# TritonDataCenter/manatee

Hardware: NVIDIA H100
Metric: snapshot_stream_gibs (higher is better)
Workload: dtype u8 / u32->u64 (mod 2^64)

## Files before the change

manatee_b200/csrc/kernels_lz4.cuh:

```cuda
#pragma once
#include <stdint.h>
#include <cuda_runtime.h>
#ifdef LZ4_PROF
#include <cstdio>
#endif
#include "../../include/manatee_gpu.h"

namespace mtz {

#define LZ4_MINMATCH     4
#define LZ4_LASTLITERALS 5
#define LZ4_MFLIMIT      12
#define LZ4_MINLENGTH    13
#define LZ4_MAXDIST      65535
#define LZ4_64KLIMIT     ((1 << 16) + (LZ4_MFLIMIT - 1))
#define LZ4_SKIPSTRENGTH 6

__device__ __forceinline__ uint32_t ld_u8(const uint8_t *p) { return *p; }

#define LZ4_SEQ_NONE 0xffffffffu
__device__ __forceinline__ uint64_t lz4_seq_pack(uint32_t m, uint32_t off, uint32_t ml)
{
	return (uint64_t)m | ((uint64_t)off << 24) | ((uint64_t)ml << 40);
}

__device__ __forceinline__ int32_t warp_lz4_decode(const uint8_t *__restrict__ src,
    uint32_t psize, uint8_t *__restrict__ dst, uint32_t lsize, int lane,
    uint64_t *__restrict__ seq = nullptr, uint32_t seq_cap = 0, uint32_t *seq_n = nullptr)
{
	uint32_t ns = 0;
	if (seq_n != nullptr && lane == 0) *seq_n = LZ4_SEQ_NONE;
	if (psize < 4u) return MTZ_ECODEC;
	const uint32_t clen = (ld_u8(src) << 24) | (ld_u8(src + 1) << 16) | (ld_u8(src + 2) << 8) | ld_u8(src + 3);
	if ((uint64_t)clen + 4u > psize || clen == 0u) return MTZ_ECODEC;
	const uint8_t *in = src + 4;
	uint32_t ip = 0, op = 0;
	const uint32_t iend = clen;

	for (;;) {
		if (ip >= iend) return MTZ_ECODEC;
		const uint32_t tok = ld_u8(in + ip++);
		uint32_t len = tok >> 4;
		if (len == 15u) {
			uint32_t s;
			do {
				if (ip >= iend) return MTZ_ECODEC;
				s = ld_u8(in + ip++);
				len += s;
			} while (s == 255u);
		}
		if (len > iend - ip || len > lsize - op) return MTZ_ECODEC;
		if ((uint32_t)lane < len) dst[op + (uint32_t)lane] = in[ip + (uint32_t)lane];
		if (len > 32u)
			for (uint32_t i = 32u + (uint32_t)lane; i < len; i += 32u) dst[op + i] = in[ip + i];
		ip += len; op += len;
		if (ip == iend) {
			if ((tok & 15u) != 0u) ns = LZ4_SEQ_NONE;
			break;
		}

		if (iend - ip < 2u) return MTZ_ECODEC;
		const uint32_t off = ld_u8(in + ip) | (ld_u8(in + ip + 1) << 8);
		ip += 2;
		if (off == 0u || off > op) return MTZ_ECODEC;
		uint32_t ml = tok & 15u;
		if (ml == 15u) {
			uint32_t s;
			do {
				if (ip >= iend) return MTZ_ECODEC;
				s = ld_u8(in + ip++);
				ml += s;
			} while (s == 255u);
		}
		ml += LZ4_MINMATCH;
		if (ml > lsize - op) return MTZ_ECODEC;
		if (seq != nullptr) {
			if (ns < seq_cap && lane == 0) seq[ns] = lz4_seq_pack(op, off, ml);
			ns++;
		}
		__syncwarp();
		const uint8_t *ref = dst + (op - off);
		if (off >= ml) {
			if ((uint32_t)lane < ml) dst[op + (uint32_t)lane] = ref[lane];
			if (ml > 32u)
				for (uint32_t i = 32u + (uint32_t)lane; i < ml; i += 32u) dst[op + i] = ref[i];
		} else {
			uint32_t r = (uint32_t)lane % off;
			const uint32_t stp = 32u % off;
			for (uint32_t i = (uint32_t)lane; i < ml; i += 32u) {
				dst[op + i] = ref[r];
				r += stp;
				if (r >= off) r -= off;
			}
		}
		op += ml;
	}
	__syncwarp();
	if (op != lsize) return MTZ_ECODEC;
	if (seq_n != nullptr && lane == 0 && ns <= seq_cap) *seq_n = ns;
	return MTZ_OK;
}

#define LZ4_THREADS 128
#define LZ4_WARPS   (LZ4_THREADS / 32)

__global__ void __launch_bounds__(LZ4_THREADS)
k2_lz4_decode(const uint8_t *__restrict__ src_base, uint8_t *__restrict__ dst_base,
    mtz_job *__restrict__ jobs, uint32_t njobs,
    const mtz_job *__restrict__ seq_jobs = nullptr, uint32_t *__restrict__ seq_n = nullptr)
{
	const int lane = threadIdx.x & 31;
	const uint32_t gw = blockIdx.x * LZ4_WARPS + (threadIdx.x >> 5);
	const uint32_t nw = gridDim.x * LZ4_WARPS;
	for (uint32_t j = gw; j < njobs; j += nw) {
		const mtz_job job = jobs[j];
		if (job.lsize == 0u) continue;
		uint64_t *seq = nullptr;
		if (seq_jobs != nullptr) seq = reinterpret_cast<uint64_t *>((uintptr_t)seq_jobs[j].dst_off);
		const int32_t st = warp_lz4_decode(src_base + job.src_off, job.src_len,
		    dst_base + job.dst_off, job.lsize, lane, seq, seq ? (job.lsize >> 3) : 0u,
		    seq ? seq_n + j : nullptr);
		if (lane == 0) {
			jobs[j].status = st;
			jobs[j].out_len = (st == MTZ_OK) ? job.lsize : 0u;
		}
	}
}



__device__ __forceinline__ uint32_t ld32u(const uint8_t *p)
{
	const uintptr_t a = (uintptr_t)p;
	const uint32_t *w = reinterpret_cast<const uint32_t *>(a & ~(uintptr_t)3);
	const uint32_t sh = (uint32_t)(a & 3u) * 8u;
	return __funnelshift_r(__ldg(w), __ldg(w + 1), sh);
}

__device__ __forceinline__ uint32_t ld32x(const uint32_t *__restrict__ base4, uint32_t x)
{
	const uint32_t i = x >> 2;
	return __funnelshift_r(__ldg(base4 + i), __ldg(base4 + i + 1u), (x & 3u) * 8u);
}

__device__ __forceinline__ uint32_t skip_dist(uint32_t x)
{
	const uint32_t T = 67u + x, q = T >> 6, r = T & 63u;
	return 64u * (q * (q - 1u) / 2u) + q * r - 3u;
}

struct TabU32 {
	uint32_t *t;
	static constexpr int LOG = 12;
	__device__ __forceinline__ void clear(int lane) const {
		for (int i = lane; i < 4096; i += 32) t[i] = 0;
	}
	__device__ __forceinline__ uint32_t get(uint32_t h) const { return t[h]; }
	__device__ __forceinline__ void set(uint32_t h, uint32_t v) const { t[h] = v; }
	__device__ __forceinline__ void set_from(uint32_t h, uint32_t v, uint32_t) const { t[h] = v; }
	__device__ __forceinline__ void tag(uint32_t h, uint32_t v) const { t[h] = v; }
	__device__ __forceinline__ uint32_t tagval(uint32_t h) const { return t[h]; }
	__device__ __forceinline__ void untag(uint32_t h, uint32_t old) const { t[h] = old; }
};
struct TabU16 {
	uint32_t *t;
	static constexpr int LOG = 13;
	__device__ __forceinline__ void clear(int lane) const {
		for (int i = lane; i < 4096; i += 32) t[i] = 0;
	}
	__device__ __forceinline__ uint32_t get(uint32_t h) const { return reinterpret_cast<uint16_t *>(t)[h]; }
	__device__ __forceinline__ void set(uint32_t h, uint32_t v) const { reinterpret_cast<uint16_t *>(t)[h] = (uint16_t)v; }
	__device__ __forceinline__ void set_from(uint32_t h, uint32_t v, uint32_t) const { reinterpret_cast<uint16_t *>(t)[h] = (uint16_t)v; }
	__device__ __forceinline__ void tag(uint32_t h, uint32_t v) const { reinterpret_cast<uint16_t *>(t)[h] = (uint16_t)v; }
	__device__ __forceinline__ uint32_t tagval(uint32_t h) const { return reinterpret_cast<uint16_t *>(t)[h]; }
	__device__ __forceinline__ void untag(uint32_t h, uint32_t old) const { reinterpret_cast<uint16_t *>(t)[h] = (uint16_t)old; }
};
struct Tab17 {
	uint32_t *t;
	static constexpr int LOG = 12;
	__device__ __forceinline__ void clear(int lane) const {
		for (int i = lane; i < 2176; i += 32) t[i] = 0;
	}
	__device__ __forceinline__ uint32_t get(uint32_t h) const {
		const uint32_t lo = reinterpret_cast<uint16_t *>(t)[h];
		const uint32_t hi = (t[2048u + (h >> 5)] >> (h & 31u)) & 1u;
		return lo | (hi << 16);
	}
	__device__ __forceinline__ void set_from(uint32_t h, uint32_t v, uint32_t old) const {
		reinterpret_cast<uint16_t *>(t)[h] = (uint16_t)v;
		if (((v ^ old) >> 16) & 1u) atomicXor(&t[2048u + (h >> 5)], 1u << (h & 31u));
	}
	__device__ __forceinline__ void set(uint32_t h, uint32_t v) const {
		const uint32_t oldhi = (t[2048u + (h >> 5)] >> (h & 31u)) & 1u;
		set_from(h, v, oldhi << 16);
	}
	__device__ __forceinline__ void tag(uint32_t h, uint32_t v) const { reinterpret_cast<uint16_t *>(t)[h] = (uint16_t)v; }
	__device__ __forceinline__ uint32_t tagval(uint32_t h) const { return reinterpret_cast<uint16_t *>(t)[h]; }
	__device__ __forceinline__ void untag(uint32_t h, uint32_t old) const { reinterpret_cast<uint16_t *>(t)[h] = (uint16_t)old; }
};

#define LZ4_TAB_BIG_WORDS     4096u
#define LZ4_TAB_COMPACT_WORDS 2176u

__device__ __forceinline__ uint32_t put_len_ext(uint8_t *dst, uint32_t op, uint32_t v, int lane)
{
	const uint32_t n255 = v / 255u;
	for (uint32_t i = (uint32_t)lane; i < n255; i += 32u) dst[op + i] = 255;
	if (lane == 0) dst[op + n255] = (uint8_t)(v - n255 * 255u);
	return op + n255 + 1u;
}

struct ExtRound {
	uint32_t wa, wb;
};

__device__ __forceinline__ ExtRound ext_load(const uint8_t *src, uint32_t ip0, uint32_t ref0,
    uint32_t iend, int lane)
{
	ExtRound e; e.wa = 0; e.wb = 0;
	const uint32_t o = 4u * (uint32_t)lane;
	if (ip0 + o + 4u <= iend) { e.wa = ld32u(src + ip0 + o); e.wb = ld32u(src + ref0 + o); }
	return e;
}

__device__ __forceinline__ uint32_t extract32(uint32_t w0, uint32_t w1, uint32_t w2, uint32_t off)
{
	return (off < 4u) ? __funnelshift_r(w0, w1, off * 8u) : __funnelshift_r(w1, w2, (off - 4u) * 8u);
}

#ifdef LZ4_PROF
#define PROF_DECL long long pt = clock64(), p_search = 0, p_b = 0, p_ext = 0, p_post = 0; unsigned n_seq = 0, n_round = 0, n_follow = 0;
#define PROF_LAP(acc) { const long long now_ = clock64(); acc += now_ - pt; pt = now_; }
#else
#define PROF_DECL
#define PROF_LAP(acc)
#endif

template <class TAB, bool DIST>
__device__ __forceinline__ uint32_t warp_lz4_encode3(const uint8_t *__restrict__ src,
    uint32_t isize, uint8_t *__restrict__ dst, uint32_t osize, uint32_t *tabmem, int lane)
{
	constexpr int LOG = TAB::LOG;
	PROF_DECL
	const uint32_t mis = (uint32_t)((uintptr_t)src & 3u);
	const uint32_t *base4 = reinterpret_cast<const uint32_t *>(src - mis);
#define LDS32(pos) ld32x(base4, (pos) + mis)
	TAB tab; tab.t = tabmem;
	const uint32_t lanebit = 1u << lane, lower = lanebit - 1u;
	tab.clear(lane);
	__syncwarp();

	uint32_t ip = 0, anchor = 0, op = 0;
	const uint32_t iend = isize;
	if (isize >= (uint32_t)LZ4_MINLENGTH) {
		const uint32_t mflimit = iend - LZ4_MFLIMIT;
		const uint32_t matchlimit = iend - LZ4_LASTLITERALS;
		ip = 1;
		bool have_pre = false;
		uint32_t vpre = 0;
		for (;;) {
			uint32_t ref = 0;
			bool to_tail = false;
			const uint32_t start = ip;
			for (uint32_t a0 = 0;; a0 += 32u) {
				uint32_t p, step;
				if (a0 == 0u) {
					p = start + (uint32_t)lane; step = 1u;
				} else {
					const uint32_t a = a0 + (uint32_t)lane;
					p = start + skip_dist(a);
					step = (67u + a) >> 6;
				}
				const bool valid = (p + step <= mflimit);
				uint32_t h = 0xffffffffu - (uint32_t)lane, cand = 0, v = 0;
				if (valid) {
					v = (a0 == 0u && have_pre) ? vpre : LDS32(p);
					h = (v * 2654435761u) >> (32 - LOG);
				}
				uint32_t oldv = 0;
				if (valid) oldv = tab.get(h);
				__syncwarp();
				if (valid) tab.tag(h, (uint32_t)lane);
				__syncwarp();
				const bool clash = valid && (tab.tagval(h) != (uint32_t)lane);
				int F, I;
				if (!__any_sync(0xffffffffu, clash)) {
					bool hit = false;
					cand = oldv;
					if (valid && (!DIST || cand + LZ4_MAXDIST >= p)) hit = (LDS32(cand) == v);
					const uint32_t hits = __ballot_sync(0xffffffffu, hit);
					const uint32_t inval = __ballot_sync(0xffffffffu, !valid);
					F = hits ? (__ffs((int)hits) - 1) : 32;
					I = inval ? (__ffs((int)inval) - 1) : 32;
					if (I < F) { to_tail = true; break; }
					if (valid) {
						if (lane <= F) tab.set_from(h, p, oldv); else tab.untag(h, oldv);
					}
				} else {
					if (valid) tab.untag(h, oldv);
					__syncwarp();
					const uint32_t all_same = __match_any_sync(0xffffffffu, h);
					const uint32_t same = all_same & lower;
					const int from = same ? (31 - __clz((int)same)) : lane;
					const uint32_t fwd = __shfl_sync(0xffffffffu, p, from);
					bool hit = false;
					if (valid) {
						cand = same ? fwd : oldv;
						if (!DIST || cand + LZ4_MAXDIST >= p) hit = (LDS32(cand) == v);
					}
					const uint32_t hits = __ballot_sync(0xffffffffu, hit);
					const uint32_t inval = __ballot_sync(0xffffffffu, !valid);
					F = hits ? (__ffs((int)hits) - 1) : 32;
					I = inval ? (__ffs((int)inval) - 1) : 32;
					if (I < F) { to_tail = true; break; }
					const uint32_t upto = (F >= 31) ? 0xffffffffu : ((2u << F) - 1u);
					const uint32_t later = all_same & ~(lanebit | lower) & upto;
					if ((lanebit & upto) && later == 0u) tab.set_from(h, p, oldv);
				}
				__syncwarp();
				if (F < 32) {
					ip = __shfl_sync(0xffffffffu, p, F);
					ref = __shfl_sync(0xffffffffu, cand, F);
					break;
				}
			}
			have_pre = false;
			PROF_LAP(p_search)
			if (to_tail) break;
#ifdef LZ4_PROF
			n_seq++;
#endif

			const uint32_t k = (uint32_t)lane + 1u;
			const bool cu_ok = (ip >= anchor + k && ref >= k);
			uint32_t ca = 0, cb = 1;
			if (cu_ok) { ca = src[ip - k]; cb = src[ref - k]; }
			uint32_t lit0 = 0;
			if (anchor + (uint32_t)lane < ip) lit0 = src[anchor + (uint32_t)lane];
			ExtRound er = ext_load(src, ip, ref, iend, lane);

			const uint32_t ip_pre = ip, ref_pre = ref;
			{
				const uint32_t ne = ~__ballot_sync(0xffffffffu, cu_ok && ca == cb);
				uint32_t n = ne ? (uint32_t)(__ffs((int)ne) - 1) : 32u;
				ip -= n; ref -= n;
				while (n == 32u) {
					bool eq = false;
					if (ip >= anchor + k && ref >= k) eq = (src[ip - k] == src[ref - k]);
					const uint32_t ne2 = ~__ballot_sync(0xffffffffu, eq);
					n = ne2 ? (uint32_t)(__ffs((int)ne2) - 1) : 32u;
					ip -= n; ref -= n;
				}
			}

			const uint32_t litlen = ip - anchor;
			uint32_t token = op++;
			if (op + litlen + (2u + 1u + LZ4_LASTLITERALS) + (litlen >> 8) > osize) return 0u;
			uint32_t tokval;
			if (litlen >= 15u) {
				tokval = 15u << 4;
				op = put_len_ext(dst, op, litlen - 15u, lane);
			} else {
				tokval = litlen << 4;
			}
			if ((uint32_t)lane < litlen) dst[op + (uint32_t)lane] = (uint8_t)lit0;
			for (uint32_t i = 32u + (uint32_t)lane; i < litlen; i += 32u) dst[op + i] = src[anchor + i];
			op += litlen;

			PROF_LAP(p_b)
			uint32_t ext_ip = ip_pre, ext_ref = ref_pre;
			for (;;) {
				if (lane == 0) {
					dst[op] = (uint8_t)((ip - ref) & 0xffu);
					dst[op + 1] = (uint8_t)((ip - ref) >> 8);
				}
				op += 2;
				anchor = ip + LZ4_MINMATCH;
				uint32_t prev31 = 0, v_end = 0, v_m2 = 0;
				for (;;) {
					const uint32_t o = 4u * (uint32_t)lane;
					const uint32_t room = (ext_ip + o < matchlimit) ? (matchlimit - ext_ip - o) : 0u;
					uint32_t n = 0;
					if (room) {
						const uint32_t x = er.wa ^ er.wb;
						n = x ? (uint32_t)((__ffs((int)x) - 1) >> 3) : 4u;
						if (n > room) n = room;
					}
					const uint32_t part = __ballot_sync(0xffffffffu, n < 4u);
					if (part) {
						const int Fp = __ffs((int)part) - 1;
						const uint32_t nf = __shfl_sync(0xffffffffu, n, Fp);
						ip = ext_ip + 4u * (uint32_t)Fp + nf;
						const uint32_t w1 = __shfl_sync(0xffffffffu, er.wa, Fp);
						uint32_t w0 = __shfl_sync(0xffffffffu, er.wa, (Fp + 31) & 31);
						uint32_t w2 = __shfl_sync(0xffffffffu, er.wa, (Fp + 1) & 31);
						if (Fp == 0) w0 = prev31;
						if (Fp == 31 && nf > 0u) w2 = (ip + 4u <= iend) ? LDS32(ext_ip + 128u) : 0u;
						v_m2 = extract32(w0, w1, w2, nf + 2u);
						v_end = extract32(w0, w1, w2, nf + 4u);
						break;
					}
					prev31 = __shfl_sync(0xffffffffu, er.wa, 31);
					ext_ip += 128u; ext_ref += 128u;
					er = ext_load(src, ext_ip, ext_ref, iend, lane);
				}
				uint32_t mlen = ip - anchor;
				if (op + (1u + LZ4_LASTLITERALS) + (mlen >> 8) > osize) return 0u;
				if (mlen >= 15u) {
					tokval += 15u;
					op = put_len_ext(dst, op, mlen - 15u, lane);
				} else {
					tokval += mlen;
				}
				if (lane == 0) dst[token] = (uint8_t)tokval;
				PROF_LAP(p_ext)

				if (ip > mflimit) { anchor = ip; to_tail = true; break; }

				const uint32_t h2 = (v_m2 * 2654435761u) >> (32 - LOG);
				if (lane == 0) tab.set(h2, ip - 2u);
				__syncwarp();
				const uint32_t hh = (v_end * 2654435761u) >> (32 - LOG);
				const uint32_t pref = tab.get(hh);
				__syncwarp();
				if (lane == 0) tab.set_from(hh, ip, pref);
				__syncwarp();
				const uint32_t np = ip + 1u + (uint32_t)lane;
				uint32_t vn = 0;
				if (np + 1u <= mflimit) vn = LDS32(np);
				ExtRound e2 = ext_load(src, ip, pref, iend, lane);
				const bool probe_hit = (!DIST || pref + LZ4_MAXDIST >= ip) &&
				    (__shfl_sync(0xffffffffu, e2.wb, 0) == v_end);
				PROF_LAP(p_post)
				if (probe_hit) {
#ifdef LZ4_PROF
					n_follow++;
#endif
					ref = pref;
					token = op++;
					tokval = 0;
					er = e2; ext_ip = ip; ext_ref = ref;
					continue;
				}
				vpre = vn; have_pre = true;
				break;
			}
			if (to_tail) break;
			anchor = ip++;
		}
	}
	{
		const uint32_t last = iend - anchor;
		if (op + last + 1u + ((last + 255u - 15u) / 255u) > osize) return 0u;
		if (last >= 15u) {
			if (lane == 0) dst[op] = (uint8_t)(15u << 4);
			op = put_len_ext(dst, op + 1u, last - 15u, lane);
		} else {
			if (lane == 0) dst[op] = (uint8_t)(last << 4);
			op += 1u;
		}
		for (uint32_t i = (uint32_t)lane; i < last; i += 32u) dst[op + i] = src[anchor + i];
		op += last;
	}
#ifdef LZ4_PROF
	if (lane == 0 && blockIdx.x == 7 && (threadIdx.x >> 5) == 1 && n_seq > 100)
		printf("K3PROF seq=%u follow=%u per-seq cycles: search %lld  B(loads+catchup+literals) %lld  ext+emit %lld  post(probe) %lld  total %lld\n",
		    n_seq, n_follow, p_search / n_seq, p_b / n_seq, p_ext / n_seq, p_post / n_seq,
		    (p_search + p_b + p_ext + p_post) / n_seq);
#endif
#undef LDS32
	return op;
}

template <bool COMPACT>
__device__ __forceinline__ uint32_t warp_zfs_lz4_compress(const uint8_t *__restrict__ src,
    uint32_t lsize, uint8_t *__restrict__ dst, uint32_t *tabmem, int lane)
{
	const uint32_t d_len = lsize - (lsize >> 3);
	if (lsize < 1024u || lsize > (16u << 20) || d_len < 4u) return lsize;
	uint32_t blk;
	if (COMPACT)
		blk = warp_lz4_encode3<Tab17, true>(src, lsize, dst + 4, d_len - 4u, tabmem, lane);
	else if (lsize < (uint32_t)LZ4_64KLIMIT)
		blk = warp_lz4_encode3<TabU16, false>(src, lsize, dst + 4, d_len - 4u, tabmem, lane);
	else
		blk = warp_lz4_encode3<TabU32, true>(src, lsize, dst + 4, d_len - 4u, tabmem, lane);
	__syncwarp();
	if (blk == 0u) return lsize;
	const uint32_t c_len = blk + 4u;
	if (c_len > d_len) return lsize;
	const uint32_t psize = (c_len + 511u) & ~511u;
	if (psize >= lsize) return lsize;
	if (lane == 0) {
		dst[0] = (uint8_t)(blk >> 24); dst[1] = (uint8_t)(blk >> 16);
		dst[2] = (uint8_t)(blk >> 8);  dst[3] = (uint8_t)blk;
	}
	for (uint32_t i = c_len + (uint32_t)lane; i < psize; i += 32u) dst[i] = 0;
	return psize;
}

template <class TAB>
struct TabRound {
	uint32_t oldv, all_same;
	bool anyclash;
};

template <class TAB>
__device__ __forceinline__ uint32_t tab_round_query(const TAB &tab, TabRound<TAB> &r, bool part,
    uint32_t h, uint32_t x, int lane)
{
	const uint32_t lanebit = 1u << lane, lower = lanebit - 1u;
	r.oldv = part ? tab.get(h) : 0u;
	__syncwarp();
	if (part) tab.tag(h, (uint32_t)lane);
	__syncwarp();
	const bool clash = part && (tab.tagval(h) != (uint32_t)lane);
	r.anyclash = __any_sync(0xffffffffu, clash);
	r.all_same = 0;
	if (!r.anyclash) return r.oldv;
	if (part) tab.untag(h, r.oldv);
	__syncwarp();
	r.all_same = __match_any_sync(0xffffffffu, h);
	const uint32_t same = r.all_same & lower;
	const int from = same ? (31 - __clz((int)same)) : lane;
	const uint32_t fwd = __shfl_sync(0xffffffffu, x, from);
	return same ? fwd : r.oldv;
}

template <class TAB>
__device__ __forceinline__ void tab_round_commit(const TAB &tab, const TabRound<TAB> &r, bool part,
    uint32_t h, uint32_t x, int upto, int lane)
{
	const uint32_t lanebit = 1u << lane, lower = lanebit - 1u;
	if (!r.anyclash) {
		if (part) {
			if (lane <= upto) tab.set_from(h, x, r.oldv); else tab.untag(h, r.oldv);
		}
	} else {
		const uint32_t uptomask = (upto >= 31) ? 0xffffffffu : ((2u << upto) - 1u);
		const uint32_t later = r.all_same & ~(lanebit | lower) & uptomask;
		if (part && (lanebit & uptomask) && later == 0u) tab.set_from(h, x, r.oldv);
	}
	__syncwarp();
}

template <class TAB, bool DIST>
__device__ __forceinline__ bool warp_lz4_certify(const uint8_t *__restrict__ src, uint32_t isize,
    const uint64_t *__restrict__ seqs, uint32_t ns, uint32_t clen, uint32_t osize,
    uint32_t *tabmem, int lane)
{
	constexpr int LOG = TAB::LOG;
	const uint32_t mis = (uint32_t)((uintptr_t)src & 3u);
	const uint32_t *base4 = reinterpret_cast<const uint32_t *>(src - mis);
#define LDS32(pos) ld32x(base4, (pos) + mis)
#define SEQ_M(s) ((uint32_t)(s) & 0xffffffu)
#define SEQ_O(s) ((uint32_t)((s) >> 24) & 0xffffu)
#define SEQ_L(s) ((uint32_t)((s) >> 40))
	const uint32_t iend = isize;
	bool bad = false;
	if (isize < (uint32_t)LZ4_MINLENGTH) {
		bad = (ns != 0u) || (isize + 1u + ((isize + 255u - 15u) / 255u) > osize) ||
		    (1u + (isize >= 15u ? 1u + (isize - 15u) / 255u : 0u) + isize != clen);
		return !bad;
	}
	const uint32_t mflimit = iend - LZ4_MFLIMIT;
	const uint32_t matchlimit = iend - LZ4_LASTLITERALS;

	{
		uint32_t op = 0, prev_e = 0;
		for (uint32_t k0 = 0; k0 < ns; k0 += 32u) {
			const uint32_t k = k0 + (uint32_t)lane;
			const bool live = k < ns;
			const uint64_t s = live ? seqs[k] : 0ull;
			const uint32_t m = SEQ_M(s), o = SEQ_O(s), ml = SEQ_L(s), e = m + ml;
			uint32_t a = __shfl_up_sync(0xffffffffu, e, 1);
			if (lane == 0) a = prev_e;
			const uint32_t litlen = m - a;
			const uint32_t lb = 1u + (litlen >= 15u ? 1u + (litlen - 15u) / 255u : 0u) + litlen;
			const uint32_t mlen = ml - LZ4_MINMATCH;
			const uint32_t mb = 2u + (mlen >= 15u ? 1u + (mlen - 15u) / 255u : 0u);
			const uint32_t tot = live ? lb + mb : 0u;
			uint32_t inc = tot;
#pragma unroll
			for (int d = 1; d < 32; d <<= 1) {
				const uint32_t t = __shfl_up_sync(0xffffffffu, inc, d);
				if (lane >= d) inc += t;
			}
			const uint32_t opk = op + inc - tot;
			if (live) {
				if (e > matchlimit) bad = true;
				else if (e < matchlimit && src[e] == src[e - o]) bad = true;
				if (litlen > 0u && m > o && src[m - 1u] == src[m - o - 1u]) bad = true;
				if (opk + 1u + litlen + (2u + 1u + LZ4_LASTLITERALS) + (litlen >> 8) > osize) bad = true;
				if (opk + lb + 2u + (1u + LZ4_LASTLITERALS) + (mlen >> 8) > osize) bad = true;
			}
			op += __shfl_sync(0xffffffffu, inc, 31);
			const uint32_t lastlive = (ns - k0 < 32u) ? (ns - k0 - 1u) : 31u;
			prev_e = __shfl_sync(0xffffffffu, e, (int)lastlive);
		}
		const uint32_t last = iend - prev_e;
		if (op + last + 1u + ((last + 255u - 15u) / 255u) > osize) bad = true;
		if (op + 1u + (last >= 15u ? 1u + (last - 15u) / 255u : 0u) + last != clen) bad = true;
	}
	if (__any_sync(0xffffffffu, bad)) return false;

	TAB tab; tab.t = tabmem;
	tab.clear(lane);
	__syncwarp();
	TabRound<TAB> rd;
	uint32_t p_lo = 0, p_hi = 0, p_sh = 0, p_v = 1;
#define CHK_EVAL() { bad = bad || (__funnelshift_r(p_lo, p_hi, p_sh) == p_v); }
#define CHK_ISSUE(chk_, pred_, v_)                                                                   \
	{                                                                                                \
		const uint32_t cx_ = (pred_) + mis;                                                          \
		p_lo = (chk_) ? __ldg(base4 + (cx_ >> 2)) : 0u;                                              \
		p_hi = (chk_) ? __ldg(base4 + (cx_ >> 2) + 1u) : 0u;                                         \
		p_sh = (cx_ & 3u) * 8u;                                                                      \
		p_v = (chk_) ? (v_) : 1u;                                                                    \
	}
	uint32_t a = 0;
	bool follow_hit = false;
	uint32_t k = 0;
	uint32_t kw = 0;
	uint64_t w_s = 0; uint32_t w_0 = 0, w_1 = 0, w_2 = 0;
	uint32_t pf_start = 0xffffffffu, pf_lo = 0, pf_hi = 0;
	bool w_init = false;
	for (;;) {
		if (__any_sync(0xffffffffu, bad)) return false;
		const bool have = k < ns;
		if (have && (!w_init || k - kw > 15u)) {
			kw = k; w_init = true;
			const uint32_t j = kw + (uint32_t)lane;
			w_s = (j < ns) ? seqs[j] : 0ull;
			const uint32_t we = SEQ_M(w_s) + SEQ_L(w_s);
			const bool wok = (j < ns) && we <= mflimit && we >= 2u;
			const uint32_t wi = (we - 2u + mis) >> 2;
			w_0 = wok ? __ldg(base4 + wi) : 0u;
			w_1 = wok ? __ldg(base4 + wi + 1u) : 0u;
			w_2 = wok ? __ldg(base4 + wi + 2u) : 0u;
		}
		const uint64_t s = have ? __shfl_sync(0xffffffffu, w_s, (int)(k - kw)) : 0ull;
		const uint32_t m = SEQ_M(s), o = SEQ_O(s), e = m + SEQ_L(s);
		uint32_t c_xx = 0, c_e = 0, c_onext = 0, c_v = 0;
		bool c_part = false, c_query = false, c_nf = false;
		int c_T = 0;
#define CHAIN_SETUP(L0)                                                                              \
		{                                                                                            \
			const int rl_ = lane - (L0);                                                             \
			const bool in_ = rl_ >= 0;                                                               \
			const uint32_t t_ = in_ ? (uint32_t)rl_ >> 1 : 0u;                                       \
			const uint32_t kk_ = k + t_;                                                             \
			const uint32_t ix_ = kk_ - kw;                   \
			const bool ex_ = in_ && kk_ < ns && ix_ <= 30u;                                          \
			const int sl_ = ex_ ? (int)ix_ : 0;                                                      \
			const uint64_t s0_ = __shfl_sync(0xffffffffu, w_s, sl_);                                 \
			const uint64_t sp_ = __shfl_sync(0xffffffffu, w_s, sl_ > 0 ? sl_ - 1 : 0);               \
			const uint64_t sn_ = __shfl_sync(0xffffffffu, w_s, sl_ + 1);                             \
			const uint32_t g0_ = __shfl_sync(0xffffffffu, w_0, sl_);                                 \
			const uint32_t g1_ = __shfl_sync(0xffffffffu, w_1, sl_);                                 \
			const uint32_t g2_ = __shfl_sync(0xffffffffu, w_2, sl_);                                 \
			c_e = SEQ_M(s0_) + SEQ_L(s0_);                                                           \
			const bool fol_ = (t_ == 0u) || (SEQ_M(s0_) == SEQ_M(sp_) + SEQ_L(sp_));                 \
			const bool good_ = ex_ && fol_ && c_e <= mflimit;                                        \
			const uint32_t bm_ = __ballot_sync(0xffffffffu, in_ && (rl_ & 1) && !good_);             \
			c_T = bm_ ? ((__ffs((int)bm_) - 1 - (L0)) >> 1) : ((32 - (L0)) >> 1);                    \
			c_part = in_ && (int)t_ < c_T;                                                           \
			c_query = c_part && (rl_ & 1);                                                           \
			c_xx = (rl_ & 1) ? c_e : c_e - 2u;                                                       \
			{                                                                                        \
				const uint32_t sh_ = ((c_e - 2u + mis) & 3u) * 8u + ((rl_ & 1) ? 16u : 0u);          \
				c_v = (sh_ < 32u) ? __funnelshift_r(g0_, g1_, sh_) : __funnelshift_r(g1_, g2_, sh_ - 32u); \
			}                                                                                        \
			c_nf = (kk_ + 1u < ns) && (SEQ_M(sn_) == c_e);                                           \
			c_onext = SEQ_O(sn_);                                                                    \
			            \
			if (c_T > 0) {                                                                           \
				pf_start = __shfl_sync(0xffffffffu, c_e, (L0) + 2 * c_T - 1) + 1u;                   \
				const uint32_t px_ = pf_start + (uint32_t)lane;                                      \
				const bool pk_ = (px_ + 4u <= iend);                                                 \
				pf_lo = pk_ ? __ldg(base4 + ((px_ + mis) >> 2)) : 0u;                                \
				pf_hi = pk_ ? __ldg(base4 + ((px_ + mis) >> 2) + 1u) : 0u;                           \
			}                                                                                        \
		}
		int c_upto = 0, c_used = 0;
		bool c_hitl = false;
#define CHAIN_FINISH(L0, pred)                                                                       \
		{                                                                                            \
			c_hitl = c_query && c_nf && ((pred) + c_onext == c_xx);                                  \
			const uint32_t mis_ = __ballot_sync(0xffffffffu, c_query && c_nf && !c_hitl);            \
			const int last_ = (L0) + 2 * c_T - 1;                                                    \
			c_upto = mis_ ? (__ffs((int)mis_) - 1) : last_;                                          \
			c_used = ((c_upto - (L0)) >> 1) + 1;                                                     \
			follow_hit = __shfl_sync(0xffffffffu, (int)c_hitl, c_upto) != 0;                         \
			a = __shfl_sync(0xffffffffu, c_e, c_upto);                                               \
		}

		bool post_done = false;
		if (!(have && follow_hit)) {
			const uint32_t start = a + 1u;
			const uint32_t pf_start_in = pf_start, pf_lo_in = pf_lo, pf_hi_in = pf_hi;
			const uint32_t target = have ? (m > start ? m : start) : 0xffffffffu;
			bool found = false, finished = false;
			uint32_t a0 = 0;
			int q1l = 32;
			uint32_t xn = 0, n_lo = 0, n_hi = 0;
			for (;;) {
				const uint32_t att = a0 + (uint32_t)lane;
				const uint32_t x = (a0 == 0u) ? start + (uint32_t)lane : xn;
				const uint32_t c_lo = n_lo, c_hi = n_hi;
				const uint32_t step = (a0 == 0u) ? 1u : ((67u + att) >> 6);
				const bool valid = (x + step <= mflimit);
				int q1, I;
				uint32_t xq1;
				if (a0 == 0u) {
					q1 = (target - start < 32u) ? (int)(target - start) : 32;
					I = (start + 1u > mflimit) ? 0 : ((mflimit - start < 32u) ? (int)(mflimit - start) : 32);
					xq1 = start + (uint32_t)q1;
				} else {
					const uint32_t cm = __ballot_sync(0xffffffffu, x >= target);
					q1 = cm ? (__ffs((int)cm) - 1) : 32;
					const uint32_t inval = __ballot_sync(0xffffffffu, !valid);
					I = inval ? (__ffs((int)inval) - 1) : 32;
					xq1 = __shfl_sync(0xffffffffu, x, q1 & 31);
				}
				q1l = q1;
				if (q1 == 32 && I == 32) {
					xn = start + skip_dist(att + 32u);
					const bool nk = (xn + 4u <= iend);
					n_lo = nk ? __ldg(base4 + ((xn + mis) >> 2)) : 0u;
					n_hi = nk ? __ldg(base4 + ((xn + mis) >> 2) + 1u) : 0u;
				}
				if (have && I <= q1 && I < 32) return false;
				if (q1 < 32 && xq1 + LZ4_MINMATCH > e) return false;
				bool part = valid && lane <= q1;
				bool query = part;
				uint32_t xx = x;
				bool ride = false;
				if (q1 < 30) {
					CHAIN_SETUP(q1 + 1)
					ride = c_T > 0;
					if (ride && c_part) { part = true; query = c_query; xx = c_xx; }
				}
				uint32_t v = 0;
				if (part) {
					if (lane > q1) v = c_v;
					else if (a0 == 0u && start == pf_start_in)
						v = __funnelshift_r(pf_lo_in, pf_hi_in, ((xx + mis) & 3u) * 8u);
					else if (a0 != 0u) v = __funnelshift_r(c_lo, c_hi, ((xx + mis) & 3u) * 8u);
					else v = LDS32(xx);
				}
				const uint32_t h = part ? ((v * 2654435761u) >> (32 - LOG)) : (0xffffffffu - (uint32_t)lane);
				const uint32_t pred = tab_round_query(tab, rd, part, h, xx, lane);
				const bool hit1 = (lane == q1) && part && (pred + o == xx);
				found = __any_sync(0xffffffffu, hit1);
				int upto = (q1 < 32) ? q1 : 31;
				bool ridehit = false;
				if (found && ride) {
					CHAIN_FINISH(q1 + 1, pred)
					upto = c_upto; ridehit = c_hitl;
					k += (uint32_t)c_used;
					post_done = true;
				}
				tab_round_commit(tab, rd, part, h, xx, upto, lane);
				CHK_EVAL()
				const bool chk = part && query && lane <= upto && !hit1 && !ridehit &&
				    (!DIST || pred + LZ4_MAXDIST >= xx);
				CHK_ISSUE(chk, pred, v)
				if (q1 < 32) break;
				if (I < 32) { finished = true; break; }
				a0 += 32u;
			}
			if (finished) break;
			if (!found) {
				uint32_t ac = a0 + (uint32_t)q1l + 1u;
				for (;;) {
					const uint32_t att = ac + (uint32_t)lane;
					const uint32_t x = start + skip_dist(att);
					const uint32_t step = (67u + att) >> 6;
					const bool part = (x + step <= mflimit) && (x + LZ4_MINMATCH <= e);
					if (!__any_sync(0xffffffffu, part)) return false;
					const uint32_t v = part ? LDS32(x) : 0u;
					const uint32_t h = part ? ((v * 2654435761u) >> (32 - LOG)) : (0xffffffffu - (uint32_t)lane);
					const uint32_t pred = tab_round_query(tab, rd, part, h, x, lane);
					const bool hit = part && (pred + o == x);
					const uint32_t hits = __ballot_sync(0xffffffffu, hit);
					const int F = hits ? (__ffs((int)hits) - 1) : 32;
					tab_round_commit(tab, rd, part, h, x, F < 32 ? F : 31, lane);
					CHK_EVAL()
					const bool chk = part && lane < F && (!DIST || pred + LZ4_MAXDIST >= x);
					CHK_ISSUE(chk, pred, v)
					if (F < 32) break;
					if (!__all_sync(0xffffffffu, part)) return false;
					ac += 32u;
				}
			}
		}
		if (!have) break;
		if (post_done) continue;
		if (e > mflimit) {
			if (k + 1u != ns) return false;
			break;
		}
		{
			CHAIN_SETUP(0)
			const uint32_t v = c_part ? c_v : 0u;
			const uint32_t h = c_part ? ((v * 2654435761u) >> (32 - LOG)) : (0xffffffffu - (uint32_t)lane);
			const uint32_t pred = tab_round_query(tab, rd, c_part, h, c_xx, lane);
			CHAIN_FINISH(0, pred)
			tab_round_commit(tab, rd, c_part, h, c_xx, c_upto, lane);
			k += (uint32_t)c_used;
			CHK_EVAL()
			const bool chk = c_query && lane <= c_upto && !c_hitl && (!DIST || pred + LZ4_MAXDIST >= c_xx);
			CHK_ISSUE(chk, pred, v)
		}
	}
#undef CHAIN_SETUP
#undef CHAIN_FINISH
	CHK_EVAL()
#undef CHK_EVAL
#undef CHK_ISSUE
#undef LDS32
#undef SEQ_M
#undef SEQ_O
#undef SEQ_L
	return !__any_sync(0xffffffffu, bad);
}

#ifndef K3_THREADS
#define K3_THREADS 128
#endif
#ifndef K3_MIN_BLOCKS
#define K3_MIN_BLOCKS 6
#endif
#define K3_WARPS (K3_THREADS / 32)
template <bool COMPACT>
__global__ void __launch_bounds__(K3_THREADS, K3_MIN_BLOCKS)
k3_lz4_encode(const uint8_t *__restrict__ src_base, uint8_t *__restrict__ dst_base,
    mtz_job *__restrict__ jobs, uint32_t njobs, const uint32_t *__restrict__ skip = nullptr)
{
	extern __shared__ uint4 s_dyn[];
	constexpr uint32_t TABW = COMPACT ? LZ4_TAB_COMPACT_WORDS : LZ4_TAB_BIG_WORDS;
	constexpr uint32_t PERW = TABW;
	const int lane = threadIdx.x & 31, warp = threadIdx.x >> 5;
	uint32_t *tab = reinterpret_cast<uint32_t *>(s_dyn) + warp * PERW;
	const uint32_t gw = blockIdx.x * K3_WARPS + (uint32_t)warp;
	const uint32_t nw = gridDim.x * K3_WARPS;
	for (uint32_t j = gw; j < njobs; j += nw) {
		if (skip != nullptr && skip[j] != 0u) continue;
		const mtz_job job = jobs[j];
		if (job.lsize == 0u) continue;
		uint32_t ps;
		if (COMPACT && (job.lsize < (uint32_t)LZ4_64KLIMIT || job.lsize > 131072u))
			ps = job.lsize;
		else
			ps = warp_zfs_lz4_compress<COMPACT>(src_base + job.src_off, job.lsize,
			    dst_base + job.dst_off, tab, lane);
		__syncwarp();
		if (lane == 0) { jobs[j].out_len = ps; jobs[j].status = MTZ_OK; }
	}
}

template <bool COMPACT>
__global__ void __launch_bounds__(K3_THREADS, K3_MIN_BLOCKS)
k3c_lz4_certify(const mtz_job *__restrict__ dec, mtz_job *__restrict__ enc,
    const uint32_t *__restrict__ seq_n, uint32_t *__restrict__ cert, uint32_t njobs)
{
	extern __shared__ uint4 s_dyn[];
	constexpr uint32_t TABW = COMPACT ? LZ4_TAB_COMPACT_WORDS : LZ4_TAB_BIG_WORDS;
	const int lane = threadIdx.x & 31, warp = threadIdx.x >> 5;
	uint32_t *tab = reinterpret_cast<uint32_t *>(s_dyn) + warp * TABW;
	const uint32_t gw = blockIdx.x * K3_WARPS + (uint32_t)warp;
	const uint32_t nw = gridDim.x * K3_WARPS;
	for (uint32_t j = gw; j < njobs; j += nw) {
		const mtz_job jd = dec[j];
		const mtz_job je = enc[j];
		const uint32_t ns = seq_n[j];
		const uint32_t lsize = je.lsize;
		uint32_t c_len = 0, psize = 0;
		bool ok = (jd.lsize != 0u && jd.lsize == lsize && jd.status == MTZ_OK && ns != LZ4_SEQ_NONE);
		const uint32_t d_len = lsize - (lsize >> 3);
		if (lsize < 1024u || lsize >= (1u << 24) || d_len < 4u) ok = false;
		if (COMPACT && (lsize < (uint32_t)LZ4_64KLIMIT || lsize > 131072u)) ok = false;
		if (ok) {
			const uint8_t *f = reinterpret_cast<const uint8_t *>((uintptr_t)jd.src_off);
			const uint32_t clen = (ld_u8(f) << 24) | (ld_u8(f + 1) << 16) | (ld_u8(f + 2) << 8) | ld_u8(f + 3);
			c_len = clen + 4u;
			psize = (c_len + 511u) & ~511u;
			if (c_len > d_len || psize >= lsize) ok = false;
			if (ok) {
				const uint8_t *src = reinterpret_cast<const uint8_t *>((uintptr_t)je.src_off);
				const uint64_t *seqs = reinterpret_cast<const uint64_t *>((uintptr_t)je.dst_off);
				if (COMPACT)
					ok = warp_lz4_certify<Tab17, true>(src, lsize, seqs, ns, clen, d_len - 4u, tab, lane);
				else if (lsize < (uint32_t)LZ4_64KLIMIT)
					ok = warp_lz4_certify<TabU16, false>(src, lsize, seqs, ns, clen, d_len - 4u, tab, lane);
				else
					ok = warp_lz4_certify<TabU32, true>(src, lsize, seqs, ns, clen, d_len - 4u, tab, lane);
			}
		}
		__syncwarp();
		if (lane == 0) {
			cert[j] = ok ? c_len : 0u;
			if (ok) { enc[j].out_len = psize; enc[j].status = MTZ_OK; }
		}
	}
}

}
```

Baseline: 23.17.

## Restructure LZ4 certify into precomputed event windows with prefetched loads

Replaces the sequential per-sequence chain/search loop in warp_lz4_certify with a windowed scheme. A warp-wide prefix sum over each 31-sequence window precomputes every hash-table event (search attempts and post-match inserts), and each round processes 32 events at once. Next-round source words are prefetched while the current round runs, and the scalar chain search only runs when a predicted hit misses. The aim is to cut serial shuffles and idle lanes during certification, in exchange for more complex index maths (a float sqrt inverse of the skip schedule) and a higher risk of subtle mismatches with the encoder's behaviour.

Result: faster. 24.71 (median of 6 runs) (+6.6%).

```diff
diff --git a/manatee_b200/csrc/kernels_lz4.cuh b/manatee_b200/csrc/kernels_lz4.cuh
--- a/manatee_b200/csrc/kernels_lz4.cuh
+++ b/manatee_b200/csrc/kernels_lz4.cuh
@@ -1,5 +1,6 @@
 #pragma once
 #include <stdint.h>
+#include <math.h>
 #include <cuda_runtime.h>
 #ifdef LZ4_PROF
 #include <cstdio>
@@ -544,6 +545,118 @@
 	__syncwarp();
 }
 
+__device__ __forceinline__ uint32_t first_attempt_at(uint32_t d)
+{
+	if (d <= 61u) return d;
+	const uint32_t d3 = d + 3u;
+	uint32_t q = (uint32_t)(0.5f + sqrtf(0.25f + (float)d3 * (1.0f / 32.0f)));
+	while (32u * q * (q - 1u) > d3) q--;
+	while (32u * q * (q + 1u) <= d3) q++;
+	return 64u * q + (d3 - 32u * q * (q - 1u) + q - 1u) / q - 67u;
+}
+
+__device__ __forceinline__ uint32_t warp_or(uint32_t v)
+{
+#ifdef MTZ_HOST_EMUL
+	for (int m = 16; m > 0; m >>= 1) v |= __shfl_xor_sync(0xffffffffu, v, m);
+	return v;
+#else
+	return __reduce_or_sync(0xffffffffu, v);
+#endif
+}
+
+#define SEQ_M(s) ((uint32_t)(s) & 0xffffffu)
+#define SEQ_O(s) ((uint32_t)((s) >> 24) & 0xffffu)
+#define SEQ_L(s) ((uint32_t)((s) >> 40))
+
+struct CertWin {
+	uint32_t d;
+	uint32_t f, cnt;
+	uint32_t x0, nsr, e;
+	uint32_t o;
+	uint32_t on;
+	uint32_t tot;
+	bool last;
+};
+
+__device__ __forceinline__ bool cert_window(CertWin &w, const uint64_t *__restrict__ seqs, uint32_t ns,
+    uint32_t k0, uint32_t prev_e, bool fol0, uint32_t skip, uint32_t mflimit, int lane)
+{
+	const uint32_t k = k0 + (uint32_t)lane;
+	const bool live = k < ns;
+	const uint64_t s = live ? seqs[k] : 0ull;
+	const uint32_t m = SEQ_M(s), e = m + SEQ_L(s);
+	uint32_t pe = __shfl_up_sync(0xffffffffu, e, 1);
+	if (lane == 0) pe = prev_e;
+	const bool fol = live && (lane == 0 ? fol0 : m == pe);
+	const uint32_t start = pe + 1u;
+	bool bad = false;
+	uint32_t nsr = 0, post = 0;
+	if (live) {
+		if (!fol) {
+			const uint32_t q = first_attempt_at(m > start ? m - start : 0u);
+			bad = start + skip_dist(q + 1u) > mflimit || start + skip_dist(q) + LZ4_MINMATCH > e;
+			nsr = q + 1u;
+		}
+		if (e <= mflimit) post = 2u;
+		else if (k + 1u != ns) bad = true;
+	} else if (k == ns && start < mflimit) {
+		nsr = first_attempt_at(mflimit - start + 1u) - 1u;
+	}
+	w.x0 = start; w.nsr = nsr; w.e = e;
+	w.o = (live && !fol) ? SEQ_O(s) : 0u;
+	w.on = __shfl_down_sync(0xffffffffu, fol ? SEQ_O(s) : 0u, 1);
+	const uint32_t sk = (lane == 0) ? skip : 0u;
+	w.cnt = nsr + post - sk;
+	uint32_t inc = w.cnt;
+#pragma unroll
+	for (int dd = 1; dd < 32; dd <<= 1) {
+		const uint32_t t = __shfl_up_sync(0xffffffffu, inc, dd);
+		if (lane >= dd) inc += t;
+	}
+	w.f = inc - w.cnt;
+	w.d = w.f - sk;
+	w.tot = __shfl_sync(0xffffffffu, inc, 30);
+	w.last = k0 + 30u >= ns;
+	return bad;
+}
+
+#define CERT_POST 0xffffffffu
+struct CertEv {
+	uint32_t x;
+	uint32_t ho;
+	uint32_t att, k, e;
+	uint32_t lo, hi;
+	bool part, query;
+};
+
+__device__ __forceinline__ CertEv cert_events(const CertWin &w, uint32_t k0, uint32_t G,
+    const uint32_t *__restrict__ base4, uint32_t mis, int lane)
+{
+	const bool mark = w.cnt != 0u && w.f >= G && w.f - G < 32u;
+	const uint32_t starts = warp_or(mark ? 1u << (w.f - G) : 0u);
+	const int c0 = __popc(__ballot_sync(0xffffffffu, w.cnt != 0u && w.f <= G));
+	const int j = (c0 - 1 + __popc(starts & ((2u << lane) - 2u))) & 31;
+	const uint32_t g = G + (uint32_t)lane;
+	const uint32_t d = __shfl_sync(0xffffffffu, w.d, j), x0 = __shfl_sync(0xffffffffu, w.x0, j);
+	const uint32_t nsr = __shfl_sync(0xffffffffu, w.nsr, j), e = __shfl_sync(0xffffffffu, w.e, j);
+	const uint32_t o = __shfl_sync(0xffffffffu, w.o, j), on = __shfl_sync(0xffffffffu, w.on, j);
+	const uint32_t i = g - d;
+	CertEv v;
+	v.part = g < w.tot;
+	v.k = k0 + (uint32_t)j; v.e = e;
+	if (i < nsr) {
+		v.x = x0 + skip_dist(i); v.att = i; v.query = true; v.ho = (i + 1u == nsr) ? o : 0u;
+	} else {
+		const bool probe = i != nsr;
+		v.x = probe ? e : e - 2u; v.att = CERT_POST; v.query = probe; v.ho = probe ? on : 0u;
+	}
+	const uint32_t xi = (v.x + mis) >> 2;
+	v.lo = v.part ? __ldg(base4 + xi) : 0u;
+	v.hi = v.part ? __ldg(base4 + xi + 1u) : 0u;
+	return v;
+}
+
 template <class TAB, bool DIST>
 __device__ __forceinline__ bool warp_lz4_certify(const uint8_t *__restrict__ src, uint32_t isize,
     const uint64_t *__restrict__ seqs, uint32_t ns, uint32_t clen, uint32_t osize,
@@ -553,9 +666,6 @@
 	const uint32_t mis = (uint32_t)((uintptr_t)src & 3u);
 	const uint32_t *base4 = reinterpret_cast<const uint32_t *>(src - mis);
 #define LDS32(pos) ld32x(base4, (pos) + mis)
-#define SEQ_M(s) ((uint32_t)(s) & 0xffffffu)
-#define SEQ_O(s) ((uint32_t)((s) >> 24) & 0xffffu)
-#define SEQ_L(s) ((uint32_t)((s) >> 40))
 	const uint32_t iend = isize;
 	bool bad = false;
 	if (isize < (uint32_t)LZ4_MINLENGTH) {
@@ -567,10 +677,13 @@
 	const uint32_t matchlimit = iend - LZ4_LASTLITERALS;
 
 	{
-		uint32_t op = 0, prev_e = 0;
-		for (uint32_t k0 = 0; k0 < ns; k0 += 32u) {
+		uint32_t op = 0, prev_e = 0, k0 = 0;
+		bool fol0 = false;
+		for (;;) {
+			CertWin w;
+			if (cert_window(w, seqs, ns, k0, prev_e, fol0, 0u, mflimit, lane)) bad = true;
 			const uint32_t k = k0 + (uint32_t)lane;
-			const bool live = k < ns;
+			const bool live = lane < 31 && k < ns;
 			const uint64_t s = live ? seqs[k] : 0ull;
 			const uint32_t m = SEQ_M(s), o = SEQ_O(s), ml = SEQ_L(s), e = m + ml;
 			uint32_t a = __shfl_up_sync(0xffffffffu, e, 1);
@@ -595,8 +708,13 @@
 				if (opk + lb + 2u + (1u + LZ4_LASTLITERALS) + (mlen >> 8) > osize) bad = true;
 			}
 			op += __shfl_sync(0xffffffffu, inc, 31);
-			const uint32_t lastlive = (ns - k0 < 32u) ? (ns - k0 - 1u) : 31u;
-			prev_e = __shfl_sync(0xffffffffu, e, (int)lastlive);
+			if (ns - k0 <= 31u) {
+				if (ns > k0) prev_e = __shfl_sync(0xffffffffu, e, (int)(ns - k0 - 1u));
+				break;
+			}
+			prev_e = __shfl_sync(0xffffffffu, e, 30);
+			fol0 = __shfl_sync(0xffffffffu, (int)(w.nsr == 0u), 31) != 0;
+			k0 += 31u;
 		}
 		const uint32_t last = iend - prev_e;
 		if (op + last + 1u + ((last + 255u - 15u) / 255u) > osize) bad = true;
@@ -618,213 +736,111 @@
 		p_sh = (cx_ & 3u) * 8u;                                                                      \
 		p_v = (chk_) ? (v_) : 1u;                                                                    \
 	}
-	uint32_t a = 0;
-	bool follow_hit = false;
-	uint32_t k = 0;
-	uint32_t kw = 0;
-	uint64_t w_s = 0; uint32_t w_0 = 0, w_1 = 0, w_2 = 0;
-	uint32_t pf_start = 0xffffffffu, pf_lo = 0, pf_hi = 0;
-	bool w_init = false;
-	for (;;) {
+#ifdef LZ4_PROF
+	unsigned n_round = 0, n_win = 1, n_p2 = 0, n_p2round = 0, n_probe = 0;
+#endif
+	CertWin w;
+	uint32_t k0 = 0;
+	cert_window(w, seqs, ns, 0u, 0u, false, 0u, mflimit, lane);
+	uint32_t G = 0;
+	CertEv cur = cert_events(w, k0, 0u, base4, mis, lane);
+	while (G < w.tot) {
 		if (__any_sync(0xffffffffu, bad)) return false;
-		const bool have = k < ns;
-		if (have && (!w_init || k - kw > 15u)) {
-			kw = k; w_init = true;
-			const uint32_t j = kw + (uint32_t)lane;
-			w_s = (j < ns) ? seqs[j] : 0ull;
-			const uint32_t we = SEQ_M(w_s) + SEQ_L(w_s);
-			const bool wok = (j < ns) && we <= mflimit && we >= 2u;
-			const uint32_t wi = (we - 2u + mis) >> 2;
-			w_0 = wok ? __ldg(base4 + wi) : 0u;
-			w_1 = wok ? __ldg(base4 + wi + 1u) : 0u;
-			w_2 = wok ? __ldg(base4 + wi + 2u) : 0u;
-		}
-		const uint64_t s = have ? __shfl_sync(0xffffffffu, w_s, (int)(k - kw)) : 0ull;
-		const uint32_t m = SEQ_M(s), o = SEQ_O(s), e = m + SEQ_L(s);
-		uint32_t c_xx = 0, c_e = 0, c_onext = 0, c_v = 0;
-		bool c_part = false, c_query = false, c_nf = false;
-		int c_T = 0;
-#define CHAIN_SETUP(L0)                                                                              \
-		{                                                                                            \
-			const int rl_ = lane - (L0);                                                             \
-			const bool in_ = rl_ >= 0;                                                               \
-			const uint32_t t_ = in_ ? (uint32_t)rl_ >> 1 : 0u;                                       \
-			const uint32_t kk_ = k + t_;                                                             \
-			const uint32_t ix_ = kk_ - kw;                   \
-			const bool ex_ = in_ && kk_ < ns && ix_ <= 30u;                                          \
-			const int sl_ = ex_ ? (int)ix_ : 0;                                                      \
-			const uint64_t s0_ = __shfl_sync(0xffffffffu, w_s, sl_);                                 \
-			const uint64_t sp_ = __shfl_sync(0xffffffffu, w_s, sl_ > 0 ? sl_ - 1 : 0);               \
-			const uint64_t sn_ = __shfl_sync(0xffffffffu, w_s, sl_ + 1);                             \
-			const uint32_t g0_ = __shfl_sync(0xffffffffu, w_0, sl_);                                 \
-			const uint32_t g1_ = __shfl_sync(0xffffffffu, w_1, sl_);                                 \
-			const uint32_t g2_ = __shfl_sync(0xffffffffu, w_2, sl_);                                 \
-			c_e = SEQ_M(s0_) + SEQ_L(s0_);                                                           \
-			const bool fol_ = (t_ == 0u) || (SEQ_M(s0_) == SEQ_M(sp_) + SEQ_L(sp_));                 \
-			const bool good_ = ex_ && fol_ && c_e <= mflimit;                                        \
-			const uint32_t bm_ = __ballot_sync(0xffffffffu, in_ && (rl_ & 1) && !good_);             \
-			c_T = bm_ ? ((__ffs((int)bm_) - 1 - (L0)) >> 1) : ((32 - (L0)) >> 1);                    \
-			c_part = in_ && (int)t_ < c_T;                                                           \
-			c_query = c_part && (rl_ & 1);                                                           \
-			c_xx = (rl_ & 1) ? c_e : c_e - 2u;                                                       \
-			{                                                                                        \
-				const uint32_t sh_ = ((c_e - 2u + mis) & 3u) * 8u + ((rl_ & 1) ? 16u : 0u);          \
-				c_v = (sh_ < 32u) ? __funnelshift_r(g0_, g1_, sh_) : __funnelshift_r(g1_, g2_, sh_ - 32u); \
-			}                                                                                        \
-			c_nf = (kk_ + 1u < ns) && (SEQ_M(sn_) == c_e);                                           \
-			c_onext = SEQ_O(sn_);                                                                    \
-			            \
-			if (c_T > 0) {                                                                           \
-				pf_start = __shfl_sync(0xffffffffu, c_e, (L0) + 2 * c_T - 1) + 1u;                   \
-				const uint32_t px_ = pf_start + (uint32_t)lane;                                      \
-				const bool pk_ = (px_ + 4u <= iend);                                                 \
-				pf_lo = pk_ ? __ldg(base4 + ((px_ + mis) >> 2)) : 0u;                                \
-				pf_hi = pk_ ? __ldg(base4 + ((px_ + mis) >> 2) + 1u) : 0u;                           \
-			}                                                                                        \
-		}
-		int c_upto = 0, c_used = 0;
-		bool c_hitl = false;
-#define CHAIN_FINISH(L0, pred)                                                                       \
-		{                                                                                            \
-			c_hitl = c_query && c_nf && ((pred) + c_onext == c_xx);                                  \
-			const uint32_t mis_ = __ballot_sync(0xffffffffu, c_query && c_nf && !c_hitl);            \
-			const int last_ = (L0) + 2 * c_T - 1;                                                    \
-			c_upto = mis_ ? (__ffs((int)mis_) - 1) : last_;                                          \
-			c_used = ((c_upto - (L0)) >> 1) + 1;                                                     \
-			follow_hit = __shfl_sync(0xffffffffu, (int)c_hitl, c_upto) != 0;                         \
-			a = __shfl_sync(0xffffffffu, c_e, c_upto);                                               \
-		}
-
-		bool post_done = false;
-		if (!(have && follow_hit)) {
-			const uint32_t start = a + 1u;
-			const uint32_t pf_start_in = pf_start, pf_lo_in = pf_lo, pf_hi_in = pf_hi;
-			const uint32_t target = have ? (m > start ? m : start) : 0xffffffffu;
-			bool found = false, finished = false;
-			uint32_t a0 = 0;
-			int q1l = 32;
-			uint32_t xn = 0, n_lo = 0, n_hi = 0;
-			for (;;) {
-				const uint32_t att = a0 + (uint32_t)lane;
-				const uint32_t x = (a0 == 0u) ? start + (uint32_t)lane : xn;
-				const uint32_t c_lo = n_lo, c_hi = n_hi;
-				const uint32_t step = (a0 == 0u) ? 1u : ((67u + att) >> 6);
-				const bool valid = (x + step <= mflimit);
-				int q1, I;
-				uint32_t xq1;
-				if (a0 == 0u) {
-					q1 = (target - start < 32u) ? (int)(target - start) : 32;
-					I = (start + 1u > mflimit) ? 0 : ((mflimit - start < 32u) ? (int)(mflimit - start) : 32);
-					xq1 = start + (uint32_t)q1;
-				} else {
-					const uint32_t cm = __ballot_sync(0xffffffffu, x >= target);
-					q1 = cm ? (__ffs((int)cm) - 1) : 32;
-					const uint32_t inval = __ballot_sync(0xffffffffu, !valid);
-					I = inval ? (__ffs((int)inval) - 1) : 32;
-					xq1 = __shfl_sync(0xffffffffu, x, q1 & 31);
-				}
-				q1l = q1;
-				if (q1 == 32 && I == 32) {
-					xn = start + skip_dist(att + 32u);
-					const bool nk = (xn + 4u <= iend);
-					n_lo = nk ? __ldg(base4 + ((xn + mis) >> 2)) : 0u;
-					n_hi = nk ? __ldg(base4 + ((xn + mis) >> 2) + 1u) : 0u;
-				}
-				if (have && I <= q1 && I < 32) return false;
-				if (q1 < 32 && xq1 + LZ4_MINMATCH > e) return false;
-				bool part = valid && lane <= q1;
-				bool query = part;
-				uint32_t xx = x;
-				bool ride = false;
-				if (q1 < 30) {
-					CHAIN_SETUP(q1 + 1)
-					ride = c_T > 0;
-					if (ride && c_part) { part = true; query = c_query; xx = c_xx; }
-				}
-				uint32_t v = 0;
-				if (part) {
-					if (lane > q1) v = c_v;
-					else if (a0 == 0u && start == pf_start_in)
-						v = __funnelshift_r(pf_lo_in, pf_hi_in, ((xx + mis) & 3u) * 8u);
-					else if (a0 != 0u) v = __funnelshift_r(c_lo, c_hi, ((xx + mis) & 3u) * 8u);
-					else v = LDS32(xx);
-				}
-				const uint32_t h = part ? ((v * 2654435761u) >> (32 - LOG)) : (0xffffffffu - (uint32_t)lane);
-				const uint32_t pred = tab_round_query(tab, rd, part, h, xx, lane);
-				const bool hit1 = (lane == q1) && part && (pred + o == xx);
-				found = __any_sync(0xffffffffu, hit1);
-				int upto = (q1 < 32) ? q1 : 31;
-				bool ridehit = false;
-				if (found && ride) {
-					CHAIN_FINISH(q1 + 1, pred)
-					upto = c_upto; ridehit = c_hitl;
-					k += (uint32_t)c_used;
-					post_done = true;
-				}
-				tab_round_commit(tab, rd, part, h, xx, upto, lane);
+#ifdef LZ4_PROF
+		n_round++;
+#endif
+		uint32_t Gn = (G + 32u < w.tot) ? G + 32u : w.tot;
+		if (!w.last && Gn + 32u > w.tot) {
+			const int jn = __popc(__ballot_sync(0xffffffffu, w.cnt != 0u && w.f <= Gn)) - 1;
+			if (jn > 0) {
+				const uint32_t pe = __shfl_sync(0xffffffffu, w.e, jn - 1);
+				const uint32_t skip = Gn - __shfl_sync(0xffffffffu, w.d, jn);
+				const bool fol = __shfl_sync(0xffffffffu, w.nsr, jn) == 0u;
+				k0 += (uint32_t)jn;
+				if (cert_window(w, seqs, ns, k0, pe, fol, skip, mflimit, lane)) bad = true;
+				Gn = 0;
+#ifdef LZ4_PROF
+				n_win++;
+#endif
+			}
+		}
+		const CertEv nx = cert_events(w, k0, Gn, base4, mis, lane);
+
+		const uint32_t v = __funnelshift_r(cur.lo, cur.hi, ((cur.x + mis) & 3u) * 8u);
+		const uint32_t h = cur.part ? ((v * 2654435761u) >> (32 - LOG)) : (0xffffffffu - (uint32_t)lane);
+		const uint32_t pred = tab_round_query(tab, rd, cur.part, h, cur.x, lane);
+		const bool hyp = cur.part && cur.ho != 0u;
+		const bool hit = hyp && pred + cur.ho == cur.x;
+		const uint32_t fails = __ballot_sync(0xffffffffu, hyp && !hit);
+		const int upto = fails ? (__ffs((int)fails) - 1) : 31;
+		tab_round_commit(tab, rd, cur.part, h, cur.x, upto, lane);
+		CHK_EVAL()
+		const bool chk = cur.part && cur.query && lane <= upto && !hit &&
+		    (!DIST || pred + LZ4_MAXDIST >= cur.x);
+		CHK_ISSUE(chk, pred, v)
+		if (fails == 0u) { cur = nx; G = Gn; continue; }
+
+		const uint32_t xf = __shfl_sync(0xffffffffu, cur.x, upto), af = __shfl_sync(0xffffffffu, cur.att, upto);
+		const uint32_t kf = __shfl_sync(0xffffffffu, cur.k, upto);
+		if (af != CERT_POST) {
+			const uint32_t of = __shfl_sync(0xffffffffu, cur.ho, upto), ef = __shfl_sync(0xffffffffu, cur.e, upto);
+			const uint32_t start = xf - skip_dist(af);
+#ifdef LZ4_PROF
+			n_p2++;
+#endif
+			for (uint32_t ac = af + 1u;; ac += 32u) {
+#ifdef LZ4_PROF
+				n_p2round++;
+#endif
+				const uint32_t att = ac + (uint32_t)lane;
+				const uint32_t x = start + skip_dist(att);
+				const uint32_t step = (67u + att) >> 6;
+				const bool part = (x + step <= mflimit) && (x + LZ4_MINMATCH <= ef);
+				if (!__any_sync(0xffffffffu, part)) return false;
+				const uint32_t v2 = part ? LDS32(x) : 0u;
+				const uint32_t h2 = part ? ((v2 * 2654435761u) >> (32 - LOG)) : (0xffffffffu - (uint32_t)lane);
+				const uint32_t pred2 = tab_round_query(tab, rd, part, h2, x, lane);
+				const bool hit2 = part && (pred2 + of == x);
+				const uint32_t hits = __ballot_sync(0xffffffffu, hit2);
+				const int F = hits ? (__ffs((int)hits) - 1) : 32;
+				tab_round_commit(tab, rd, part, h2, x, F < 32 ? F : 31, lane);
 				CHK_EVAL()
-				const bool chk = part && query && lane <= upto && !hit1 && !ridehit &&
-				    (!DIST || pred + LZ4_MAXDIST >= xx);
-				CHK_ISSUE(chk, pred, v)
-				if (q1 < 32) break;
-				if (I < 32) { finished = true; break; }
-				a0 += 32u;
-			}
-			if (finished) break;
-			if (!found) {
-				uint32_t ac = a0 + (uint32_t)q1l + 1u;
-				for (;;) {
-					const uint32_t att = ac + (uint32_t)lane;
-					const uint32_t x = start + skip_dist(att);
-					const uint32_t step = (67u + att) >> 6;
-					const bool part = (x + step <= mflimit) && (x + LZ4_MINMATCH <= e);
-					if (!__any_sync(0xffffffffu, part)) return false;
-					const uint32_t v = part ? LDS32(x) : 0u;
-					const uint32_t h = part ? ((v * 2654435761u) >> (32 - LOG)) : (0xffffffffu - (uint32_t)lane);
-					const uint32_t pred = tab_round_query(tab, rd, part, h, x, lane);
-					const bool hit = part && (pred + o == x);
-					const uint32_t hits = __ballot_sync(0xffffffffu, hit);
-					const int F = hits ? (__ffs((int)hits) - 1) : 32;
-					tab_round_commit(tab, rd, part, h, x, F < 32 ? F : 31, lane);
-					CHK_EVAL()
-					const bool chk = part && lane < F && (!DIST || pred + LZ4_MAXDIST >= x);
-					CHK_ISSUE(chk, pred, v)
-					if (F < 32) break;
-					if (!__all_sync(0xffffffffu, part)) return false;
-					ac += 32u;
-				}
-			}
-		}
-		if (!have) break;
-		if (post_done) continue;
-		if (e > mflimit) {
-			if (k + 1u != ns) return false;
-			break;
-		}
-		{
-			CHAIN_SETUP(0)
-			const uint32_t v = c_part ? c_v : 0u;
-			const uint32_t h = c_part ? ((v * 2654435761u) >> (32 - LOG)) : (0xffffffffu - (uint32_t)lane);
-			const uint32_t pred = tab_round_query(tab, rd, c_part, h, c_xx, lane);
-			CHAIN_FINISH(0, pred)
-			tab_round_commit(tab, rd, c_part, h, c_xx, c_upto, lane);
-			k += (uint32_t)c_used;
-			CHK_EVAL()
-			const bool chk = c_query && lane <= c_upto && !c_hitl && (!DIST || pred + LZ4_MAXDIST >= c_xx);
-			CHK_ISSUE(chk, pred, v)
-		}
-	}
-#undef CHAIN_SETUP
-#undef CHAIN_FINISH
+				const bool chk2 = part && lane < F && (!DIST || pred2 + LZ4_MAXDIST >= x);
+				CHK_ISSUE(chk2, pred2, v2)
+				if (F < 32) break;
+				if (!__all_sync(0xffffffffu, part)) return false;
+			}
+			k0 = kf;
+			if (cert_window(w, seqs, ns, k0, 0u, true, 0u, mflimit, lane)) bad = true;
+		} else {
+#ifdef LZ4_PROF
+			n_probe++;
+#endif
+			k0 = kf + 1u;
+			if (cert_window(w, seqs, ns, k0, xf, false, 0u, mflimit, lane)) bad = true;
+		}
+#ifdef LZ4_PROF
+		n_win++;
+#endif
+		G = 0;
+		cur = cert_events(w, k0, 0u, base4, mis, lane);
+	}
 	CHK_EVAL()
 #undef CHK_EVAL
 #undef CHK_ISSUE
 #undef LDS32
+	const bool ok = !__any_sync(0xffffffffu, bad);
+#ifdef LZ4_PROF
+	if (lane == 0)
+		printf("K3CPROF lsize=%u seqs=%u ok=%d rounds=%u windows=%u phase2=%u phase2_rounds=%u probe_misses=%u\n",
+		    isize, ns, (int)ok, n_round, n_win, n_p2, n_p2round, n_probe);
+#endif
+	return ok;
+}
 #undef SEQ_M
 #undef SEQ_O
 #undef SEQ_L
-	return !__any_sync(0xffffffffu, bad);
-}
+#undef CERT_POST
 
 #ifndef K3_THREADS
 #define K3_THREADS 128
```
